# simonrw/rust-tensorflow-serving2

Measured on AMD Instinct MI355X. Metric: Predict RPCs/sec + p50 latency, ResNet-50 batch=1/32 at 1/2/4/8 MI355X, higher is better.
Workload: dtype bf16

## Files before the change

rust_tensorflow_serving2_amd/graph/fused.py:

```python
from __future__ import annotations

import os
from typing import Dict, List, Optional, Sequence, Set, Tuple

import numpy as np
import torch
import torch.nn.functional as F

from ..utils import tensors as T
from . import ops as O
from .ir import Graph, Node
from .placement import to_device, zeros

BF16 = torch.bfloat16


def _const(g: Graph, ref) -> Optional[torch.Tensor]:
    n = g.nodes.get(ref[0])
    if n is None or n.op != "Const" or n.value is None:
        return None
    v = n.value[ref[1]] if ref[1] < len(n.value) else None
    return v if isinstance(v, torch.Tensor) else None


# ... 686 lines not shown
        if not (self.use_hip and x.is_cuda and x.dim() == 4):
            return pool(ctx, node, conv(ctx, node, [x]))
        from ..ops import ACT, hip
        pt, pb, pl, pr = conv.pads_for(x.shape[1], x.shape[2])
        hc = (x.shape[1] + pt + pb - conv.kh) // conv.sh + 1
        wc = (x.shape[2] + pl + pr - conv.kw) // conv.sw + 1
        if pool.padding == "SAME":
            (ppt, ppb), (ppl, ppr) = O.tf_same_pads(hc, 3, 2), O.tf_same_pads(wc, 3, 2)
        else:
            ppt = ppb = ppl = ppr = 0
        kw = {}
        if pool.post is not None:
            sc, sh, act = pool.post
            kw = dict(post_scale=sc, post_shift=sh, post_act=ACT[act])
        x = x.contiguous() if x.dtype == torch.bfloat16 else x.float().contiguous()
        return [hip().stem_pool(x, conv.w, conv.b, pt, pb, pl, pr, ACT[conv.act],
                                ppt, ppb, ppl, ppr, **kw)]


O.OPS["_StemPool"] = _impl_op

CHAIN_SHAPES_ALL = {(64, 256, 64), (64, 256, 128), (128, 512, 128), (128, 512, 256)}
CHAIN_SHAPES_STAGE1 = {(64, 256, 64), (64, 256, 128)}
CHAIN_SHAPES_DEFAULT = CHAIN_SHAPES_ALL


class ChainConv:

    children = ("a", "b")

    def __init__(self, a: FusedConv, b: FusedConv):
        self.a, self.b = a, b
        self.use_hip = a.use_hip and b.use_hip
        self.name = a.name

    def __call__(self, ctx, node, ins):
        x = O.to_torch(ins[0])
        res = O.to_torch(ins[1]) if len(ins) > 1 else None
        a, b = self.a, self.b

        def split():
            y1 = a(ctx, node, ins)[0]
            return [y1, b(ctx, node, [y1])[0]]
        if not (self.use_hip and x.is_cuda and x.dim() == 4 and x.shape[-1] == a.cin):
            return split()
        from ..ops import ACT, hip, tuned_choice
        xb = _to_bf16(x).contiguous()
        rb = None if res is None else _to_bf16(res).contiguous()

        def chained():
            return list(hip().conv_chain(xb, a.w, a.b, rb, ACT[a.act], b.w, b.b, ACT[b.act]))
        key = ("chain", tuple(x.shape), a.cout, b.cout, res is not None, a.act, b.act)
        dflt = 1 if (a.cin, a.cout, b.cout) in CHAIN_SHAPES_STAGE1 else 0
        pick = tuned_choice(key, {1: chained, 0: split}, default=dflt)
        return chained() if pick == 1 else split()


O.OPS["_ChainConv"] = _impl_op
O.OPS["_FusedMatMulLN"] = _impl_op

_PASSTHROUGH = ("Identity", "Squeeze", "Reshape")


def fuse_classifier_head(g, order, fed, fetch_refs, device, opts):
    c = _Ctx(g, order, fed, fetch_refs, device, opts)

    def single(node) -> bool:
        return node.name not in c.fetch_nodes and len(c.cons.get(node.name, [])) == 1

    def walk(ref, chain):
        n = g.nodes.get(ref[0])
        while n is not None and n.op in _PASSTHROUGH and ref[1] == 0 and single(n) and n.inputs:
            chain.append(n)
            ref = n.inputs[0]
            n = g.nodes.get(ref[0])
        return ref, n
# ... 344 lines not shown
            g.nodes[cn].inputs[pos] = new_ref
        p.ctrl = _merge_ctrl([p, bn] + ([out_node] if out_node is not bn else []))
        del g.nodes[bn.name]
        if out_node is not bn:
            del g.nodes[out_node.name]
        c.refresh()


def _chainable_1x1(impl) -> bool:
    return (isinstance(impl, FusedConv) and impl.kh == 1 and impl.kw == 1 and impl.sh == 1 and impl.sw == 1 and
            not impl.c4 and impl.post is None and impl.act in ("relu", "none") and
            (impl.padding != "EXPLICIT" or not any(impl.pads)))


def fuse_conv_chain(g, order, fed, fetch_refs, device, opts):
    import os
    mode = os.environ.get("TFSERVE_CONV_CHAIN", "1")
    shapes = CHAIN_SHAPES_STAGE1 if os.environ.get("TFSERVE_CONV_CHAIN_SHAPES") == "stage1" else CHAIN_SHAPES_ALL
    c = _Ctx(g, order, fed, fetch_refs, device, opts)
    if mode == "0" or (not c.use_hip and mode != "force"):
        return
    for name in order:
        p = g.nodes.get(name)
        if p is None or p.op != "_FusedConv2D" or name in c.fetch_nodes:
            continue
        a = p.attrs["_impl"]
        if not _chainable_1x1(a):
            continue
        cons = c.cons.get(name, [])
        if any(i != 0 for _c, _p, i in cons):
            continue
        bs = [g.nodes[cn] for cn, pos, _i in cons
              if pos == 0 and g.nodes[cn].op == "_FusedConv2D" and len(g.nodes[cn].inputs) == 1 and
              cn not in c.fetch_nodes and _chainable_1x1(g.nodes[cn].attrs["_impl"])]
        if len(bs) != 1:
            continue
        bnode = bs[0]
        b = bnode.attrs["_impl"]
        if b.cin != a.cout or (a.cin, a.cout, b.cout) not in shapes:
            continue
        chain = ChainConv(a, b)
        p.op = "_ChainConv"
        p.attrs = {"_impl": chain}
        for cn, pos, _i in c.cons.get(bnode.name, []):
            g.nodes[cn].inputs[pos] = (name, 1)
        p.ctrl = _merge_ctrl([p, bnode])
        del g.nodes[bnode.name]
        c.refresh()


def default_passes(options=None):
    from .patterns import bert_passes, late_passes
    return [fuse_pools, fuse_softmax_argmax] + bert_passes() + [fuse_conv, fuse_dual_conv, fuse_post_activation,
                                                                 fuse_stem_pool, fuse_matmul,
                                                                 fuse_classifier_head, fuse_dense_softmax,
                                                                 fuse_conv_chain] + late_passes() + \
        [fuse_matmul_layernorm, defer_layernorm, release_weight_sources]
```

rust_tensorflow_serving2_amd/kernels/bindings.cpp:

```cpp
#include <cstdlib>
#include <algorithm>
#include <torch/extension.h>
#include <ATen/hip/impl/HIPGuardImplMasqueradingAsCUDA.h>
#include <ATen/hip/impl/HIPStreamMasqueradingAsCUDA.h>

#include "launch.h"
#include "cgemm.h"

namespace {

using torch::Tensor;

hipStream_t cur_stream(const Tensor& t) {
  return c10::hip::getCurrentHIPStreamMasqueradingAsCUDA(t.device().index()).stream();
}

void check(hipError_t e, const char* what) {
  TORCH_CHECK(e == hipSuccess, what, ": ", hipGetErrorString(e));
}

bool is_cgemm_cfg(int64_t cfg) {
  return cfg >= 0 && cfg < (1 << 20) && tfsk::cgemm_cfg_id(int(cfg));
}

// ... 407 lines not shown
  const int Hc = (H + PT + PB - 7) / 2 + 1, Wc = (W + PL + PR - 7) / 2 + 1;
  TORCH_CHECK(Hc >= 1 && Wc >= 1, "stem_pool: input smaller than the filter");
  const int Hp = (Hc + PPT + PPB - 3) / 2 + 1, Wp = (Wc + PPL + PPR - 3) / 2 + 1;
  TORCH_CHECK(Hp >= 1 && Wp >= 1, "stem_pool: conv output smaller than the pool window");
  Tensor y = torch::empty({N, Hp, Wp, cout}, x.options().dtype(at::kBFloat16));
  const float* sc = nullptr;
  const float* sh = nullptr;
  if (post_scale.has_value()) {
    TORCH_CHECK(post_shift.has_value(), "post_scale needs post_shift");
    need(*post_scale, at::kFloat, "post_scale");
    need(*post_shift, at::kFloat, "post_shift");
    TORCH_CHECK(post_scale->numel() == cout && post_shift->numel() == cout, "post scale / shift must have cout entries");
    sc = post_scale->data_ptr<float>();
    sh = post_shift->data_ptr<float>();
  }
  check(tfsk::stem_pool_launch(xin.data_ptr(), xb16, bf16p(w), int(w.size(1)), bias.data_ptr<float>(), bf16p_mut(y), N,
                               H, W, C, cout, int(PT), int(PL), Hc, Wc, int(PPT), int(PPL), Hp, Wp, int(act), sc, sh,
                               int(post_act), cur_stream(x)), "stem_pool");
  return y;
}

std::vector<Tensor> conv_chain(const Tensor& x, const Tensor& w1, const Tensor& b1,
                               const c10::optional<Tensor>& residual, int64_t act1, const Tensor& w2,
                               const Tensor& b2, int64_t act2) {
  need(x, at::kBFloat16, "x");
  need(w1, at::kBFloat16, "w1");
  need(w2, at::kBFloat16, "w2");
  need(b1, at::kFloat, "b1");
  need(b2, at::kFloat, "b2");
  TORCH_CHECK(x.dim() == 4, "conv_chain: x must be NHWC");
  const int K1 = x.size(3), N1 = w1.size(0), N2 = w2.size(0);
  TORCH_CHECK(w1.dim() == 2 && w2.dim() == 2 && w1.size(1) >= K1 && w2.size(1) >= N1 && w1.size(1) % 8 == 0 &&
                  w2.size(1) % 8 == 0, "conv_chain: w1 [N1][>= K1], w2 [N2][>= N1]");
  TORCH_CHECK(tfsk::conv_chain_supported(K1, N1, N2), "conv_chain: unsupported shape K1=", K1, " N1=", N1, " N2=", N2);
  TORCH_CHECK(b1.numel() == N1 && b2.numel() == N2, "conv_chain: bias sizes");
  TORCH_CHECK(w1.device() == x.device() && w2.device() == x.device() && b1.device() == x.device() &&
                  b2.device() == x.device(), "conv_chain: tensors on different devices");
  const uint16_t* rp = nullptr;
  if (residual.has_value()) {
    need(*residual, at::kBFloat16, "residual");
    TORCH_CHECK(residual->dim() == 4 && residual->size(0) == x.size(0) && residual->size(1) == x.size(1) &&
                    residual->size(2) == x.size(2) && residual->size(3) == N1, "conv_chain: residual [n][h][w][N1]");
    rp = bf16p(*residual);
  }
  c10::hip::HIPGuardMasqueradingAsCUDA guard(x.device());
  const int M = x.size(0) * x.size(1) * x.size(2);
  Tensor y1 = torch::empty({x.size(0), x.size(1), x.size(2), N1}, x.options());
  Tensor y2 = torch::empty({x.size(0), x.size(1), x.size(2), N2}, x.options());
  check(tfsk::conv_chain_launch(bf16p(x), bf16p(w1), int(w1.size(1)), b1.data_ptr<float>(), rp, bf16p_mut(y1),
                                bf16p(w2), int(w2.size(1)), b2.data_ptr<float>(), bf16p_mut(y2), M, K1, N1, N2,
                                int(act1), int(act2), cur_stream(x)),
        "conv_chain");
  return {y1, y2};
}

Tensor global_avgpool(const Tensor& x, const c10::optional<Tensor>& out) {
  need(x, at::kBFloat16, "x");
  TORCH_CHECK(x.dim() == 4 && x.size(3) % 8 == 0, "global_avgpool: NHWC with C % 8 == 0");
  c10::hip::HIPGuardMasqueradingAsCUDA guard(x.device());
  const int N = x.size(0), HW = x.size(1) * x.size(2), C = x.size(3);
  Tensor y = out.has_value() ? *out : torch::empty({N, C}, x.options());
  need(y, at::kBFloat16, "out");
  check(tfsk::global_avgpool_nhwc_launch(bf16p(x), bf16p_mut(y), N, HW, C, cur_stream(x)), "gap");
  return y;
}

std::vector<Tensor> softmax_argmax(const Tensor& logits, bool want_probs, bool want_classes,
                                   const c10::optional<Tensor>& probs_out,
                                   const c10::optional<Tensor>& classes_out) {
  TORCH_CHECK(logits.is_cuda() && logits.dim() >= 1 && logits.stride(-1) == 1 &&
                  (logits.is_contiguous() || logits.dim() == 2),
              "logits must be a GPU tensor with unit column stride (contiguous, or 2-D with a row stride)");
  const bool bf = logits.scalar_type() == at::kBFloat16;
  TORCH_CHECK(bf || logits.scalar_type() == at::kFloat, "logits must be f32 or bf16");
// ... 243 lines not shown
                "mask strides exceed the mask tensor");
    mb = mask_bias->data_ptr<float>();
  }
  Tensor y = out.has_value() ? *out : torch::empty({B, S, heads * D}, qkv.options());
  need(y, at::kBFloat16, "out");
  check(tfsk::attention_launch(bf16p(qkv), mb, bf16p_mut(y), B, S, heads, D, float(scale), mask_bstride,
                               mask_qstride, cur_stream(qkv)),
        "attention");
  return y;
}

}

PYBIND11_MODULE(TORCH_EXTENSION_NAME, m) {
  m.doc() = "gfx950 HIP kernels (MFMA implicit-GEMM conv/GEMM, attention, norms, pooling)";
  m.def("conv2d", &conv2d, "NHWC implicit-GEMM conv (+bias +residual +act)", py::arg("x"), py::arg("w"),
        py::arg("bias"), py::arg("residual"), py::arg("kh"), py::arg("kw"), py::arg("sh"), py::arg("sw"),
        py::arg("pt"), py::arg("pb"), py::arg("pl"), py::arg("pr"), py::arg("act") = 0, py::arg("cfg") = 0,
        py::arg("out") = py::none(), py::arg("out_f32") = false, py::arg("splits") = 1,
        py::arg("post_scale") = py::none(), py::arg("post_shift") = py::none(), py::arg("post_act") = 0,
        py::arg("out2") = py::none(), py::arg("post_only") = false);
  m.def("conv_chain", &conv_chain, "expand 1x1 (+residual, act) -> next reduce 1x1 (+act) in one kernel",
        py::arg("x"), py::arg("w1"), py::arg("b1"), py::arg("residual"), py::arg("act1"), py::arg("w2"),
        py::arg("b2"), py::arg("act2"));
  m.def("conv_chain_supported", [](int64_t k1, int64_t n1, int64_t n2) {
    return tfsk::conv_chain_supported(int(k1), int(n1), int(n2));
  });
  m.def("conv2d_dual", &conv2d_dual, "act(conv1x1(h) + conv1x1_stride(x) + bias) as one K-concatenated GEMM",
        py::arg("h"), py::arg("x"), py::arg("w"), py::arg("bias"), py::arg("sh"), py::arg("sw"), py::arg("act") = 0,
        py::arg("cfg") = 36, py::arg("out") = py::none(), py::arg("splits") = 1,
        py::arg("post_scale") = py::none(), py::arg("post_shift") = py::none(), py::arg("post_act") = 0,
        py::arg("out2") = py::none(), py::arg("post_only") = false);
  m.def("linear_lnx", &linear_lnx,
        "GEMM whose A / residual rows are LayerNorm inputs (statistics as partials), optionally "
        "returning its own rows' partials: {y, partials}",
        py::arg("x"), py::arg("w"), py::arg("bias"), py::arg("residual"), py::arg("act"), py::arg("cfg"),
        py::arg("out_f32") = false, py::arg("out") = py::none(), py::arg("a_st") = py::none(),
        py::arg("a_colsum") = py::none(), py::arg("a_eps") = 1e-12, py::arg("r_st") = py::none(),
        py::arg("r_gamma") = py::none(), py::arg("r_beta") = py::none(), py::arg("r_eps") = 1e-12,
        py::arg("stats") = false);
  m.def("linear", &linear,"x @ w^T (+bias +residual +act)", py::arg("x"), py::arg("w"), py::arg("bias"),
        py::arg("residual") = py::none(), py::arg("act") = 0, py::arg("cfg") = 0, py::arg("out_f32") = false,
        py::arg("alpha") = 1.0, py::arg("out") = py::none(), py::arg("splits") = 1);
  m.def("stem_pool", &stem_pool, py::arg("x"), py::arg("w"), py::arg("bias"), py::arg("pt"), py::arg("pb"),
        py::arg("pl"), py::arg("pr"), py::arg("act"), py::arg("ppt"), py::arg("ppb"), py::arg("ppl"), py::arg("ppr"),
        py::arg("post_scale") = py::none(), py::arg("post_shift") = py::none(), py::arg("post_act") = 0);
  m.def("maxpool", &maxpool, py::arg("x"), py::arg("kh"), py::arg("kw"), py::arg("sh"), py::arg("sw"),
        py::arg("pt"), py::arg("pb"), py::arg("pl"), py::arg("pr"), py::arg("out") = py::none(),
        py::arg("post_scale") = py::none(), py::arg("post_shift") = py::none(), py::arg("post_act") = 0);
  m.def("global_avgpool", &global_avgpool, py::arg("x"), py::arg("out") = py::none());
// ... 97 lines not shown
```

rust_tensorflow_serving2_amd/kernels/chain.hip:

```cpp
#include "gemm_common.h"

namespace tfsk {
namespace {

using namespace gemm;

struct ChainArgs {
  const uint16_t* x;
  const uint16_t* w1;
  const float* b1;
  const uint16_t* res;
  uint16_t* y1;
  const uint16_t* w2;
  const float* b2;
  uint16_t* y2;
  int M, ldw1, ldw2;
  float lo1, lo2;
};

constexpr int kBM = 64, kNT = 256, kStgLd = 68;

template <int K1, int N1, int N2>
struct CH {
  static constexpr int KT1 = K1 / KT, KT2 = N1 / KT;
  static constexpr int A_BYTES = KT1 * kBM * KT * 2;
  static constexpr int W1_BYTES = KT1 * N1 * KT * 2;
  static constexpr int P1 = A_BYTES + W1_BYTES;
  static constexpr int CHAIN = KT2 * kBM * KT * 2;
  static constexpr int STG = 4 * 16 * kStgLd * 4;
  static constexpr int S2 = N2 <= 128 ? 3 : 2;
  static constexpr int W2_SLOT = N2 * KT * 2;
  static constexpr int RING_OFF = CHAIN;
  static constexpr int P23 = CHAIN + (STG > S2 * W2_SLOT ? STG : S2 * W2_SLOT);
  static constexpr int LDS = P1 > P23 ? P1 : P23;
  static constexpr int WN1 = N1 / 4, TN1 = WN1 / 16, U1 = WN1 / 64;
  static constexpr int WN2 = N2 / 2, TN2 = WN2 / 16;
  static constexpr int UW2 = WN2 < 64 ? WN2 : 64, U2 = WN2 / UW2;
  static constexpr int APW = KT1 * (kBM / 8) / 4, W1PW = KT1 * (N1 / 8) / 4, W2PW = N2 / 32;
  static_assert(K1 % KT == 0 && N1 % 256 == 0 && N2 % 64 == 0, "chain shape");
  static_assert(LDS <= 160 * 1024, "LDS budget");
  static_assert((S2 - 2) * W2PW < 64, "vmcnt range");
};

template <int K1, int N1, int N2>
__global__ __launch_bounds__(256, 1) void conv_chain_kernel(ChainArgs p) {
  using G = CH<K1, N1, N2>;
  extern __shared__ __attribute__((aligned(16))) char smem[];
  typedef __attribute__((address_space(3))) void* lds_ptr_t;
  const int tid = threadIdx.x, lane = tid & 63;
  const int wid = __builtin_amdgcn_readfirstlane(tid >> 6);
  const int fr = lane & 15, fq = lane >> 4;
  const int prow = lane >> 3;
  const uint32_t kc = uint32_t(((lane & 7) ^ prow) * 8);
  const int m0 = xcd_remap(blockIdx.x, gridDim.x) * kBM;
  const int M = p.M;

  const __amdgpu_buffer_rsrc_t rsX = __builtin_amdgcn_make_buffer_rsrc(
      const_cast<uint16_t*>(p.x), 0, int(long(M) * K1 * 2), 0x00020000);
  const __amdgpu_buffer_rsrc_t rsW1 = __builtin_amdgcn_make_buffer_rsrc(
      const_cast<uint16_t*>(p.w1), 0, int(long(N1) * p.ldw1 * 2), 0x00020000);
  const __amdgpu_buffer_rsrc_t rsW2 = __builtin_amdgcn_make_buffer_rsrc(
      const_cast<uint16_t*>(p.w2), 0, int(long(N2) * p.ldw2 * 2), 0x00020000);

#pragma unroll
  for (int j = 0; j < G::APW; ++j) {
    const int q = wid * G::APW + j;
    const int kt = q / (kBM / 8), pc = q % (kBM / 8);
    const int m = m0 + pc * 8 + prow;
    const uint32_t v = m < M ? (uint32_t(m) * K1 + uint32_t(kt * KT) + kc) * 2u : kOOB;
    __builtin_amdgcn_raw_ptr_buffer_load_lds(rsX, (lds_ptr_t)(smem + kt * kBM * KT * 2 + pc * 1024), 16, v, 0, 0, 0);
  }
#pragma unroll
  for (int j = 0; j < G::W1PW; ++j) {
    const int q = wid * G::W1PW + j;
    const int kt = q / (N1 / 8), pc = q % (N1 / 8);
    const int n = pc * 8 + prow;
    const uint32_t v = (uint32_t(n) * uint32_t(p.ldw1) + uint32_t(kt * KT) + kc) * 2u;
    __builtin_amdgcn_raw_ptr_buffer_load_lds(rsW1, (lds_ptr_t)(smem + G::A_BYTES + kt * N1 * KT * 2 + pc * 1024), 16,
                                             v, 0, 0, 0);
  }

  const int c8 = lane & 7, rl = lane >> 3;
  float4 bias1[G::U1][2];
#pragma unroll
  for (int c = 0; c < G::U1; ++c) {
    const int n = wid * G::WN1 + c * 64 + c8 * 8;
    bias1[c][0] = *reinterpret_cast<const float4*>(p.b1 + n);
    bias1[c][1] = *reinterpret_cast<const float4*>(p.b1 + n + 4);
  }
  const __amdgpu_buffer_rsrc_t rsR = __builtin_amdgcn_make_buffer_rsrc(
      const_cast<uint16_t*>(p.res), 0, p.res ? int(long(M) * N1 * 2) : 0, 0x00020000);
  u32x4 rr[4][G::U1][2];
#pragma unroll
// ... 165 lines not shown
#pragma unroll
      for (int k = 0; k < IT2; ++k) {
        const int item = lane + 64 * k;
        const int rloc = item / CPR2, cc = item % CPR2;
        const float* src = stg + rloc * kStgLd + cc * 8;
        const float4 lo = *reinterpret_cast<const float4*>(src);
        const float4 hi = *reinterpret_cast<const float4*>(src + 4);
        const int n = wn2 * G::WN2 + c * G::UW2 + cc * 8;
        const u32x4 b0 = b2v[c][k][0], b1 = b2v[c][k][1];
        auto f = [](uint32_t u) { return __uint_as_float(u); };
        u32x4 ov;
        ov.x = pack_bf16x2(fmaxf(lo.x + f(b0.x), p.lo2), fmaxf(lo.y + f(b0.y), p.lo2));
        ov.y = pack_bf16x2(fmaxf(lo.z + f(b0.z), p.lo2), fmaxf(lo.w + f(b0.w), p.lo2));
        ov.z = pack_bf16x2(fmaxf(hi.x + f(b1.x), p.lo2), fmaxf(hi.y + f(b1.y), p.lo2));
        ov.w = pack_bf16x2(fmaxf(hi.z + f(b1.z), p.lo2), fmaxf(hi.w + f(b1.w), p.lo2));
        const int m = m0 + wm2 * 32 + i * 16 + rloc;
        __builtin_amdgcn_raw_buffer_store_b128(ov, rsY2, m < M ? (uint32_t(m) * N2 + uint32_t(n)) * 2u : kOOB, 0, 0);
      }
      __builtin_amdgcn_wave_barrier();
    }
  }
}

template <int K1, int N1, int N2>
hipError_t launch_chain(const ChainArgs& a, hipStream_t s) {
  using G = CH<K1, N1, N2>;
  hipError_t e = ensure_dyn_lds(reinterpret_cast<const void*>(&conv_chain_kernel<K1, N1, N2>), G::LDS);
  if (e != hipSuccess) return e;
  const int tiles = (a.M + kBM - 1) / kBM;
  hipLaunchKernelGGL((conv_chain_kernel<K1, N1, N2>), dim3(tiles), dim3(kNT), G::LDS, s, a);
  return hipGetLastError();
}

}

bool conv_chain_supported(int K1, int N1, int N2) {
  return (K1 == 64 && N1 == 256 && (N2 == 64 || N2 == 128)) || (K1 == 128 && N1 == 512 && (N2 == 128 || N2 == 256));
}

hipError_t conv_chain_launch(const uint16_t* x, const uint16_t* w1, int ldw1, const float* b1, const uint16_t* res,
                             uint16_t* y1, const uint16_t* w2, int ldw2, const float* b2, uint16_t* y2, int M, int K1,
                             int N1, int N2, int act1, int act2, hipStream_t s) {
  if (M <= 0) return hipSuccess;
  if (!conv_chain_supported(K1, N1, N2) || ldw1 < K1 || ldw1 % 8 || ldw2 < N1 || ldw2 % 8) return hipErrorInvalidValue;
  if ((act1 != kActNone && act1 != kActRelu) || (act2 != kActNone && act2 != kActRelu)) return hipErrorInvalidValue;
  if (long(M) * N1 * 2 >= 0x7fffffffL) return hipErrorInvalidValue;
  ChainArgs a{x, w1, b1, res, y1, w2, b2, y2, M, ldw1, ldw2, act1 == kActRelu ? 0.f : -INFINITY,
              act2 == kActRelu ? 0.f : -INFINITY};
  if (K1 == 64 && N1 == 256 && N2 == 64) return launch_chain<64, 256, 64>(a, s);
  if (K1 == 64 && N1 == 256 && N2 == 128) return launch_chain<64, 256, 128>(a, s);
  if (K1 == 128 && N1 == 512 && N2 == 128) return launch_chain<128, 512, 128>(a, s);
  return launch_chain<128, 512, 256>(a, s);
}

}
```

rust_tensorflow_serving2_amd/kernels/halo.hip:

```cpp
#include <algorithm>
#include <type_traits>

#include "gemm_common.h"
#include "cgemm.h"

namespace tfsk {

namespace {

using namespace gemm;

__device__ __forceinline__ int halo_key(int lin) { return lin & 7; }

template <int BM, int BN, int WGM, int WGN, int HR, int S_>
struct HG {
  static constexpr int NW = WGM * WGN, NT = 64 * NW;
  static constexpr int WM = BM / WGM, WN = BN / WGN;
  static constexpr int TM = WM / 16, TN = WN / 16;
  static constexpr int HPW = HR / (8 * NW);
  static constexpr int BPW = BN / (8 * NW);
  static constexpr int S = S_;
  static_assert(S == 3 || S == 9, "ring depth must divide the 9 taps (static slots)");
  static constexpr int HALO_B = HR * 128;
  static constexpr int B_B = BN * 128;
// ... 337 lines not shown
  trace_stamp(p, 2);

  halo_epilogue<BM, BN, G::NT, G::TM, G::TN, G::WM, G::WN>(p, acc, smem, h0, w0, img, n0, wm, wn, tid, bias0,
                                                              bias1);
  trace_stamp(p, 3);
}

constexpr int kPersistBM = 128, kPersistBN = 64, kPersistHR = 192;
struct HPs {
  static constexpr int BM = kPersistBM, BN = kPersistBN, HR = kPersistHR;
  static constexpr int WGM = 4, WGN = 2, NW = 8, NT = 512;
  static constexpr int WM = BM / WGM, WN = BN / WGN, TM = WM / 16, TN = WN / 16;
  static constexpr int HPW = HR / (8 * NW), BPW = BN / (8 * NW);
  static constexpr int B_B = BN * 128, HALO_B = HR * 128;
  static constexpr int CB_LD = BN + 8;
  static constexpr int STG_B = BM * CB_LD * 2;
  static constexpr int OFF_HALO = 9 * B_B, OFF_STG = OFF_HALO + 2 * HALO_B;
  static constexpr int LDS = OFF_STG + STG_B;
  static constexpr int kStores = BM * (BN / 8) / NT;
  static_assert(HPW * 8 * NW == HR && BPW == 1 && kStores * NT == BM * (BN / 8), "persistent halo split");
  static_assert(LDS <= 160 * 1024, "LDS budget");
};

__global__ __launch_bounds__(512, 1) void halo_persist_kernel(IGemmArgs p, int ntiles) {
  using G = HPs;
  constexpr int BM = G::BM, BN = G::BN;
  extern __shared__ __attribute__((aligned(16))) char smem_raw[];
  char* const smem = reinterpret_cast<char*>(smem_raw);
  typedef __attribute__((address_space(3))) void* lds_ptr_t;

  const int TH = p.TH, TW = p.TW, HW2 = TW + 2;
  const int Ho = p.Ho, Wo = p.Wo, H = p.H, W = p.W, C = p.C;
  const int tph = (Ho + TH - 1) / TH, tpw = (Wo + TW - 1) / TW;
  const int TI = p.TI > 1 ? p.TI : 1, nimg = p.M / (Ho * Wo);
  const int HB = (TH + 2) * HW2, hrows = TI * HB;
  const int tid = threadIdx.x, lane = tid & 63;
  const int wid = __builtin_amdgcn_readfirstlane(tid >> 6);
  const int wm = wid / G::WGN, wn = wid % G::WGN;
  const int prow = lane >> 3;
  const int fr = lane & 15, fq = lane >> 4;

  const __amdgpu_buffer_rsrc_t rsA =
      __builtin_amdgcn_make_buffer_rsrc(const_cast<void*>(p.a), 0, int(p.a_bytes), 0x00020000);
  const __amdgpu_buffer_rsrc_t rsB =
      __builtin_amdgcn_make_buffer_rsrc(const_cast<uint16_t*>(p.b), 0, int(p.b_bytes), 0x00020000);
  const __amdgpu_buffer_rsrc_t rsO =
      __builtin_amdgcn_make_buffer_rsrc(p.out, 0, int(long(p.M) * p.ldc * 2), 0x00020000);
  const bool use_b = p.bias != nullptr;
  const __amdgpu_buffer_rsrc_t rsb =
      __builtin_amdgcn_make_buffer_rsrc(const_cast<float*>(p.bias), 0, use_b ? BN * 4 : 0, 0x00020000);

  float bj[G::TN];
#pragma unroll
  for (int j = 0; j < G::TN; ++j)
    bj[j] = __uint_as_float(__builtin_amdgcn_raw_buffer_load_b32(rsb, uint32_t(wn * G::WN + j * 16 + fr) * 4u, 0, 0));
  const float alpha = p.alpha;
  gemm::wait_vmcnt<0>();

  {
    const uint32_t kc = uint32_t(((lane & 7) ^ prow) * 8);
    const int n = wid * 8 + prow;
    const uint32_t boff = (uint32_t(n) * uint32_t(p.ldb) + kc) * 2u;
#pragma unroll
// ... 25 lines not shown
  };

  int hrow0[G::TM], kpx0[G::TM];
#pragma unroll
  for (int i = 0; i < G::TM; ++i) {
    const int px = wm * G::WM + i * 16 + fr;
    const int ii = px / (TH * TW), p2 = px - ii * (TH * TW);
    const int ph = p2 / TW;
    hrow0[i] = px < TI * TH * TW ? ii * HB + ph * HW2 + (p2 - ph * TW) : 0;
    kpx0[i] = px;
  }
  const uint32_t rb0 = uint32_t(((wn * G::WN + fr) * KT + ((fq ^ (fr & 7)) * 8)) * 2);
  const uint32_t rb1 = uint32_t(((wn * G::WN + fr) * KT + (((4 + fq) ^ (fr & 7)) * 8)) * 2);
  constexpr int CPRB = BN / 8;
  uint16_t* const Cb = reinterpret_cast<uint16_t*>(smem + G::OFF_STG);

  int t = blockIdx.x;
  if (t < ntiles) issue_halo(t, 0);
  for (int k = 0; t < ntiles; t += gridDim.x, ++k) {
    const int b = k & 1;
    if (k == 0) gemm::wait_vmcnt<0>();
    else gemm::wait_vmcnt<G::kStores>();
    gemm::lds_barrier();
    const int tn = t + gridDim.x;
    if (tn < ntiles) issue_halo(tn, b ^ 1);
    __builtin_amdgcn_sched_barrier(0);

    f32x4 acc[G::TM][G::TN];
#pragma unroll
    for (int i = 0; i < G::TM; ++i)
#pragma unroll
      for (int j = 0; j < G::TN; ++j) acc[i][j] = f32x4{0.f, 0.f, 0.f, 0.f};
    const char* hb = smem + G::OFF_HALO + b * G::HALO_B;
    struct TapFrags {
      bf16x8 a[2][G::TM], b[2][G::TN];
    };
    auto load_tap = [&](TapFrags& f, int u) __attribute__((always_inline)) {
      const int tap_off = (u / 3) * HW2 + (u % 3), tap_key = (u / 3) * TW + (u % 3);
      const char* sb = smem + u * G::B_B;
#pragma unroll
      for (int kk = 0; kk < 2; ++kk) {
#pragma unroll
        for (int i = 0; i < G::TM; ++i) {
          const int hr = hrow0[i] + tap_off;
          const uint32_t addr = uint32_t(hr) * 128u + ((uint32_t((kk * 4 + fq) ^ halo_key(kpx0[i] + tap_key))) << 4);
          f.a[kk][i] = *reinterpret_cast<const bf16x8*>(hb + addr);
        }
#pragma unroll
        for (int j = 0; j < G::TN; ++j)
          f.b[kk][j] = *reinterpret_cast<const bf16x8*>(sb + (kk ? rb1 : rb0) + j * 16 * KT * 2);
      }
    };
    TapFrags fr2[2];
    load_tap(fr2[0], 0);
#pragma unroll
    for (int u = 0; u < 9; ++u) {
      __builtin_amdgcn_sched_barrier(0);
      if (u < 8) load_tap(fr2[(u + 1) & 1], u + 1);
      __builtin_amdgcn_sched_barrier(0);
      const TapFrags& f = fr2[u & 1];
#pragma unroll
      for (int kk = 0; kk < 2; ++kk)
#pragma unroll
        for (int i = 0; i < G::TM; ++i)
#pragma unroll
          for (int j = 0; j < G::TN; ++j)
            acc[i][j] = __builtin_amdgcn_mfma_f32_16x16x32_bf16(f.a[kk][i], f.b[kk][j], acc[i][j], 0, 0, 0);
    }
    __builtin_amdgcn_sched_barrier(0);

    auto stage = [&](auto act_tag) __attribute__((always_inline)) {
      constexpr int ACT = decltype(act_tag)::value;
#pragma unroll
      for (int i = 0; i < G::TM; ++i)
#pragma unroll
        for (int j = 0; j < G::TN; ++j)
#pragma unroll
          for (int r = 0; r < 4; ++r) {
            const float v = act_fn<ACT>(acc[i][j][r] * alpha + bj[j] + 0.f);
            Cb[(wm * G::WM + i * 16 + fq * 4 + r) * G::CB_LD + wn * G::WN + j * 16 + fr] =
                __builtin_bit_cast(uint16_t, static_cast<__bf16>(v));
          }
    };
    switch (p.act) {
      case kActRelu: stage(std::integral_constant<int, kActRelu>{}); break;
      case kActGeluTanh: stage(std::integral_constant<int, kActGeluTanh>{}); break;
      case kActTanh: stage(std::integral_constant<int, kActTanh>{}); break;
      default: stage(std::integral_constant<int, kActNone>{}); break;
    }
    gemm::lds_barrier();
    {
      int r_ = t;
      const int tw = r_ % tpw;
      r_ /= tpw;
      const int th = r_ % tph;
      const int img = (r_ / tph) * TI;
      const int h0 = th * TH, w0 = tw * TW;
#pragma unroll
      for (int it = 0; it < G::kStores; ++it) {
        const int c = tid + it * G::NT, row = c / CPRB, ch = c - row * CPRB;
        int m = -1;
        if (row < TI * TH * TW) {
          const int ii = row / (TH * TW), r2 = row - ii * (TH * TW);
          const int ph = r2 / TW, pw = r2 - ph * TW;
          const int h = h0 + ph, w = w0 + pw;
          if (h < Ho && w < Wo && img + ii < nimg) m = ((img + ii) * Ho + h) * Wo + w;
        }
        const uint32_t off = m >= 0 ? (uint32_t(m) * uint32_t(p.ldc) + uint32_t(ch * 8)) * 2u : kOOB;
        const u32x4 v = *reinterpret_cast<const u32x4*>(Cb + row * G::CB_LD + ch * 8);
        __builtin_amdgcn_raw_buffer_store_b128(v, rsO, off, 0, 0);
      }
    }
  }
  gemm::wait_vmcnt<0>();
}



bool pick_block(int Ho, int Wo, int BM, int HR, int& TH, int& TW) {
  long best_tiles = -1, best_halo = 0;
  for (int tw = 1; tw <= Wo; ++tw) {
    int th = BM / tw < Ho ? BM / tw : Ho;
    while (th >= 1 && (th + 2) * (tw + 2) > HR) --th;
    if (th < 1) continue;
    const int nh = (Ho + th - 1) / th, nw = (Wo + tw - 1) / tw;
    const int bh = (Ho + nh - 1) / nh, bw = (Wo + nw - 1) / nw;
    const long tiles = long(nh) * nw;
    const long halo = long(bh + 2) * (bw + 2);
    if (best_tiles < 0 || tiles < best_tiles || (tiles == best_tiles && halo < best_halo)) {
      best_tiles = tiles;
      best_halo = halo;
      TH = bh;
      TW = bw;
    }
  }
  return best_tiles > 0;
}
// ... 32 lines not shown

hipError_t launch_halo_persist(const IGemmArgs& a0, hipStream_t s) {
  using G = HPs;
  IGemmArgs a = a0;
  if (a.C != KT || a.N != G::BN || a.splits > 1 || a.residual != nullptr || a.out2 != nullptr || a.out_f32 ||
      a.out == nullptr || a.act == kActGeluErf || epi_f32_env() || a.counters != nullptr || a.ldc % 8)
    return hipErrorInvalidValue;
  if (long(a.M) * a.ldc * 2 >= 0x7fffffffL) return hipErrorInvalidValue;
  if (!pick_block(a.Ho, a.Wo, G::BM, G::HR, a.TH, a.TW)) return hipErrorInvalidValue;
  a.TI = pick_images(a, G::BM, G::HR);
  const int nimg = a.M / (a.Ho * a.Wo);
  const long tiles = long((nimg + a.TI - 1) / a.TI) * ((a.Ho + a.TH - 1) / a.TH) * ((a.Wo + a.TW - 1) / a.TW);
  if (tiles == 0) return hipSuccess;
  if (tiles >= (1L << 30)) return hipErrorInvalidValue;
  static int cus = 0;
  if (cus == 0) {
    int dev = 0, n = 0;
    if (hipGetDevice(&dev) != hipSuccess || hipDeviceGetAttribute(&n, hipDeviceAttributeMultiprocessorCount, dev) !=
                                                hipSuccess || n <= 0)
      n = 256;
    cus = n;
  }
  const int grid = int(tiles < cus ? tiles : cus);
  hipError_t e = ensure_dyn_lds(reinterpret_cast<const void*>(&halo_persist_kernel), G::LDS);
  if (e != hipSuccess) return e;
  hipLaunchKernelGGL(halo_persist_kernel, dim3(unsigned(grid)), dim3(G::NT), G::LDS, s, a, int(tiles));
  return hipGetLastError();
}

constexpr int kHBM[kNumHaloConfigs] = {256, 128, 128, 64, 256, 64, 64, 128, 256, 128, 128};
constexpr int kHBN[kNumHaloConfigs] = {64, 128, 64, 64, 128, 128, 64, 64, 64, 64, 64};
constexpr int kHHR[kNumHaloConfigs] = {320, 192, 192, 128, 320, 128, 128, 192, 320, 192, 192};

int halo_cfg_index(int cfg) {
  if (cfg >= kHaloCfgBase && cfg < kHaloCfgBase + kNumHaloConfigs) return cfg - kHaloCfgBase;
  if (cfg >= kHaloPfCfgBase && cfg < kHaloPfCfgBase + kNumHaloConfigs) return cfg - kHaloPfCfgBase;
  return -1;
}

}

long halo_tiles(const IGemmArgs& a0, int cfg) {
  IGemmArgs a = a0;
  a.epi_f32 = epi_f32_env();
  if (cfg == kHaloPersistCfg) return 0;
  const int c = halo_cfg_index(cfg);
  if (c < 0) return 0;
  if (!pick_block(a.Ho, a.Wo, kHBM[c], kHHR[c], a.TH, a.TW)) return 0;
  const int nimg = a.M / (a.Ho * a.Wo);
// ... 51 lines not shown
```

rust_tensorflow_serving2_amd/kernels/launch.h:

```cpp
#pragma once
#include <hip/hip_runtime.h>
#include <stdint.h>

namespace tfsk {

struct IGemmArgs {
  const void* a;
  const uint16_t* b;
  int M, N, K;
  int lda, ldb;
  int H, W, C, KH, KW, SH, SW, PT, PL, Ho, Wo;
  const float* bias;
  const uint16_t* residual;
  int ldr;
  int act;
  void* out;
  int ldc;
  int out_f32;
  float alpha;
  int splits;
  int kt_per_split;
  float* ws;
  int64_t a_bytes;
  int64_t b_bytes;
// ... 30 lines not shown
int64_t splitk_counters_pending();
int64_t splitk_counters_captured_in_use();

enum AMode : int { kADense = 0, kAIm2col = 1, kAStemF32 = 2, kAStem7x7x3 = 3, kAC4 = 4, kADual = 5 };

hipError_t ingest_c4_launch(const float* x, uint16_t* y, int64_t pixels, int C, hipStream_t stream);

hipError_t ingest_c4_pad_launch(const float* x, uint16_t* y, int N, int H, int W, int C, int Hp, int Wp, int pt,
                               int pl, hipStream_t stream);

hipError_t splitk_reduce_launch(const IGemmArgs& args, hipStream_t stream);

constexpr int kNumIGemmConfigs = 17;
int igemm_config_bm(int cfg);
int igemm_config_bn(int cfg);
int igemm_config_stages(int cfg);
int igemm_config_bk(int cfg);
hipError_t igemm_launch(const IGemmArgs& args, int a_mode, int cfg, hipStream_t stream);

hipError_t stem_pool_launch(const void* x, bool x_bf16, const uint16_t* w, int ldw, const float* bias, uint16_t* y,
                            int N, int H, int W, int C, int cout, int pt, int pl, int Hc, int Wc, int ppt, int ppl,
                            int Hp, int Wp, int act, const float* pscale, const float* pshift, int pact,
                            hipStream_t s);
bool conv_chain_supported(int K1, int N1, int N2);
hipError_t conv_chain_launch(const uint16_t* x, const uint16_t* w1, int ldw1, const float* b1, const uint16_t* res,
                             uint16_t* y1, const uint16_t* w2, int ldw2, const float* b2, uint16_t* y2, int M, int K1,
                             int N1, int N2, int act1, int act2, hipStream_t s);
hipError_t maxpool_nhwc_launch(const uint16_t* x, uint16_t* y, int N, int H, int W, int C,
                               int KH, int KW, int SH, int SW, int PT, int PL, int Ho, int Wo,
                               hipStream_t stream, const float* scale = nullptr, const float* shift = nullptr,
                               int act = 0);
hipError_t global_avgpool_nhwc_launch(const uint16_t* x, uint16_t* y, int N, int HW, int C,
                                      hipStream_t stream);
hipError_t classifier_head_launch(const uint16_t* x, const uint16_t* w, const float* bias, float* ws,
                                  float* probs, int64_t* classes, int M, int HW, int K, int Np, int N,
                                  hipStream_t s, int* counter = nullptr, float* probs_h = nullptr,
                                  int64_t* classes_h = nullptr);
size_t classifier_head_ws_floats(int M, int K, int Np);
bool classifier_head_one_launch(int M, int HW, int K, int Np, int N);
hipError_t dense_softmax_launch(const float* x, int ldx, const uint16_t* w, int ldw, const float* bias,
                                float* probs, int rows, int N, int K, hipStream_t s);
hipError_t key_mask_adder_launch(const void* m, int is_int, float one, float scale, float* out, int64_t n,
                                 hipStream_t s);
hipError_t softmax_argmax_launch(const void* logits, int in_bf16, float* probs, int64_t* classes,
                                 int rows, int cols, long ld, hipStream_t stream);
hipError_t cast_f32_bf16_launch(const float* x, uint16_t* y, int64_t n, hipStream_t stream);
hipError_t cast_bf16_f32_launch(const uint16_t* x, float* y, int64_t n, hipStream_t stream);
int epi_f32_env();
hipError_t h2d_rows_launch(const void* host, void* dev, int64_t bytes, hipStream_t stream);

// ... 28 lines not shown
```

Before: 55980.

## Chain dual-source 1x1 projection conv into following reduce conv

Extends the chained 1x1 conv kernel so the first GEMM can take two input sources, K-concatenated (the dual conv that merges the bottleneck expand with the shortcut projection). The first stage-1 block's projection output then feeds the next block's reduce conv in one kernel, saving a launch and a round trip of the 256-channel intermediate through memory. It is enabled by default for the (128,256,64) shape through the tuned choice. The halo persistent kernel also gains a compile-time trace variant so the untraced path carries no trace branches.

```diff
diff --git a/rust_tensorflow_serving2_amd/graph/fused.py b/rust_tensorflow_serving2_amd/graph/fused.py
--- a/rust_tensorflow_serving2_amd/graph/fused.py
+++ b/rust_tensorflow_serving2_amd/graph/fused.py
@@ -732,6 +732,7 @@
 
 CHAIN_SHAPES_ALL = {(64, 256, 64), (64, 256, 128), (128, 512, 128), (128, 512, 256)}
 CHAIN_SHAPES_STAGE1 = {(64, 256, 64), (64, 256, 128)}
+CHAIN_SHAPES_DUAL = {(128, 256, 64)}
 CHAIN_SHAPES_DEFAULT = CHAIN_SHAPES_ALL
 
 
@@ -739,19 +740,25 @@
 
     children = ("a", "b")
 
-    def __init__(self, a: FusedConv, b: FusedConv):
+    def __init__(self, a, b: FusedConv):
         self.a, self.b = a, b
+        self.dual = isinstance(a, FusedDualConv)
         self.use_hip = a.use_hip and b.use_hip
         self.name = a.name
+        if self.dual:
+            from types import SimpleNamespace
+            self.subs = [(a, SimpleNamespace(op="_FusedDualConv")), (b, SimpleNamespace(op="_FusedConv2D"))]
 
     def __call__(self, ctx, node, ins):
         x = O.to_torch(ins[0])
-        res = O.to_torch(ins[1]) if len(ins) > 1 else None
         a, b = self.a, self.b
 
         def split():
             y1 = a(ctx, node, ins)[0]
             return [y1, b(ctx, node, [y1])[0]]
+        if self.dual:
+            return self._call_dual(x, O.to_torch(ins[1]), split)
+        res = O.to_torch(ins[1]) if len(ins) > 1 else None
         if not (self.use_hip and x.is_cuda and x.dim() == 4 and x.shape[-1] == a.cin):
             return split()
         from ..ops import ACT, hip, tuned_choice
@@ -762,6 +769,21 @@
             return list(hip().conv_chain(xb, a.w, a.b, rb, ACT[a.act], b.w, b.b, ACT[b.act]))
         key = ("chain", tuple(x.shape), a.cout, b.cout, res is not None, a.act, b.act)
         dflt = 1 if (a.cin, a.cout, b.cout) in CHAIN_SHAPES_STAGE1 else 0
+        pick = tuned_choice(key, {1: chained, 0: split}, default=dflt)
+        return chained() if pick == 1 else split()
+
+    def _call_dual(self, h, x, split):
+        a, b = self.a, self.b
+        if not (self.use_hip and h.is_cuda and h.dim() == 4 and x.dim() == 4 and h.shape[:3] == x.shape[:3] and
+                h.shape[-1] == a.c1 and x.shape[-1] == a.c2):
+            return split()
+        from ..ops import ACT, hip, tuned_choice
+        hb, xb = _to_bf16(h).contiguous(), _to_bf16(x).contiguous()
+
+        def chained():
+            return list(hip().conv_chain(hb, a.w, a.b, None, ACT[a.act], b.w, b.b, ACT[b.act], x2=xb))
+        key = ("chain", tuple(h.shape), a.cout, b.cout, ("dual", a.c2), a.act, b.act)
+        dflt = 1 if (a.c1 + a.c2, a.cout, b.cout) in CHAIN_SHAPES_DUAL else 0
         pick = tuned_choice(key, {1: chained, 0: split}, default=dflt)
         return chained() if pick == 1 else split()
 
@@ -1152,10 +1174,14 @@
         return
     for name in order:
         p = g.nodes.get(name)
-        if p is None or p.op != "_FusedConv2D" or name in c.fetch_nodes:
+        if p is None or p.op not in ("_FusedConv2D", "_FusedDualConv") or name in c.fetch_nodes:
             continue
         a = p.attrs["_impl"]
-        if not _chainable_1x1(a):
+        dual = p.op == "_FusedDualConv"
+        if dual:
+            if not (a.use_hip and a.sh == a.sw == 1 and a.post is None and a.act in ("relu", "none")):
+                continue
+        elif not _chainable_1x1(a):
             continue
         cons = c.cons.get(name, [])
         if any(i != 0 for _c, _p, i in cons):
@@ -1167,7 +1193,8 @@
             continue
         bnode = bs[0]
         b = bnode.attrs["_impl"]
-        if b.cin != a.cout or (a.cin, a.cout, b.cout) not in shapes:
+        shape = (a.c1 + a.c2 if dual else a.cin, a.cout, b.cout)
+        if b.cin != a.cout or shape not in (CHAIN_SHAPES_DUAL if dual else shapes):
             continue
         chain = ChainConv(a, b)
         p.op = "_ChainConv"
diff --git a/rust_tensorflow_serving2_amd/kernels/bindings.cpp b/rust_tensorflow_serving2_amd/kernels/bindings.cpp
--- a/rust_tensorflow_serving2_amd/kernels/bindings.cpp
+++ b/rust_tensorflow_serving2_amd/kernels/bindings.cpp
@@ -453,17 +453,30 @@
 
 std::vector<Tensor> conv_chain(const Tensor& x, const Tensor& w1, const Tensor& b1,
                                const c10::optional<Tensor>& residual, int64_t act1, const Tensor& w2,
-                               const Tensor& b2, int64_t act2) {
+                               const Tensor& b2, int64_t act2, const c10::optional<Tensor>& x2) {
   need(x, at::kBFloat16, "x");
   need(w1, at::kBFloat16, "w1");
   need(w2, at::kBFloat16, "w2");
   need(b1, at::kFloat, "b1");
   need(b2, at::kFloat, "b2");
   TORCH_CHECK(x.dim() == 4, "conv_chain: x must be NHWC");
-  const int K1 = x.size(3), N1 = w1.size(0), N2 = w2.size(0);
+  const bool dual = x2.has_value();
+  const int Ka = x.size(3);
+  const uint16_t* x2p = nullptr;
+  if (dual) {
+    need(*x2, at::kBFloat16, "x2");
+    TORCH_CHECK(x2->dim() == 4 && x2->size(0) == x.size(0) && x2->size(1) == x.size(1) && x2->size(2) == x.size(2),
+                "conv_chain: x2 must have x's n, h, w");
+    TORCH_CHECK(Ka % 64 == 0 && x2->size(3) % 64 == 0 && x2->size(3) > 0,
+                "conv_chain: both sources' channels must be multiples of 64");
+    TORCH_CHECK(x2->device() == x.device(), "conv_chain: tensors on different devices");
+    x2p = bf16p(*x2);
+  }
+  const int K1 = Ka + (dual ? int(x2->size(3)) : 0), N1 = w1.size(0), N2 = w2.size(0);
   TORCH_CHECK(w1.dim() == 2 && w2.dim() == 2 && w1.size(1) >= K1 && w2.size(1) >= N1 && w1.size(1) % 8 == 0 &&
                   w2.size(1) % 8 == 0, "conv_chain: w1 [N1][>= K1], w2 [N2][>= N1]");
-  TORCH_CHECK(tfsk::conv_chain_supported(K1, N1, N2), "conv_chain: unsupported shape K1=", K1, " N1=", N1, " N2=", N2);
+  TORCH_CHECK(tfsk::conv_chain_supported(K1, N1, N2, dual), "conv_chain: unsupported shape K1=", K1, " N1=", N1,
+              " N2=", N2, dual ? " (dual)" : "");
   TORCH_CHECK(b1.numel() == N1 && b2.numel() == N2, "conv_chain: bias sizes");
   TORCH_CHECK(w1.device() == x.device() && w2.device() == x.device() && b1.device() == x.device() &&
                   b2.device() == x.device(), "conv_chain: tensors on different devices");
@@ -480,7 +493,7 @@
   Tensor y2 = torch::empty({x.size(0), x.size(1), x.size(2), N2}, x.options());
   check(tfsk::conv_chain_launch(bf16p(x), bf16p(w1), int(w1.size(1)), b1.data_ptr<float>(), rp, bf16p_mut(y1),
                                 bf16p(w2), int(w2.size(1)), b2.data_ptr<float>(), bf16p_mut(y2), M, K1, N1, N2,
-                                int(act1), int(act2), cur_stream(x)),
+                                int(act1), int(act2), cur_stream(x), x2p, Ka),
         "conv_chain");
   return {y1, y2};
 }
@@ -770,10 +783,10 @@
         py::arg("out2") = py::none(), py::arg("post_only") = false);
   m.def("conv_chain", &conv_chain, "expand 1x1 (+residual, act) -> next reduce 1x1 (+act) in one kernel",
         py::arg("x"), py::arg("w1"), py::arg("b1"), py::arg("residual"), py::arg("act1"), py::arg("w2"),
-        py::arg("b2"), py::arg("act2"));
-  m.def("conv_chain_supported", [](int64_t k1, int64_t n1, int64_t n2) {
-    return tfsk::conv_chain_supported(int(k1), int(n1), int(n2));
-  });
+        py::arg("b2"), py::arg("act2"), py::arg("x2") = py::none());
+  m.def("conv_chain_supported", [](int64_t k1, int64_t n1, int64_t n2, bool dual) {
+    return tfsk::conv_chain_supported(int(k1), int(n1), int(n2), dual);
+  }, py::arg("k1"), py::arg("n1"), py::arg("n2"), py::arg("dual") = false);
   m.def("conv2d_dual", &conv2d_dual, "act(conv1x1(h) + conv1x1_stride(x) + bias) as one K-concatenated GEMM",
         py::arg("h"), py::arg("x"), py::arg("w"), py::arg("bias"), py::arg("sh"), py::arg("sw"), py::arg("act") = 0,
         py::arg("cfg") = 36, py::arg("out") = py::none(), py::arg("splits") = 1,
diff --git a/rust_tensorflow_serving2_amd/kernels/chain.hip b/rust_tensorflow_serving2_amd/kernels/chain.hip
--- a/rust_tensorflow_serving2_amd/kernels/chain.hip
+++ b/rust_tensorflow_serving2_amd/kernels/chain.hip
@@ -7,6 +7,7 @@
 
 struct ChainArgs {
   const uint16_t* x;
+  const uint16_t* x2;
   const uint16_t* w1;
   const float* b1;
   const uint16_t* res;
@@ -15,6 +16,7 @@
   const float* b2;
   uint16_t* y2;
   int M, ldw1, ldw2;
+  int K1a;
   float lo1, lo2;
 };
 
@@ -42,7 +44,7 @@
   static_assert((S2 - 2) * W2PW < 64, "vmcnt range");
 };
 
-template <int K1, int N1, int N2>
+template <int K1, int N1, int N2, bool DUAL = false>
 __global__ __launch_bounds__(256, 1) void conv_chain_kernel(ChainArgs p) {
   using G = CH<K1, N1, N2>;
   extern __shared__ __attribute__((aligned(16))) char smem[];
@@ -55,8 +57,11 @@
   const int m0 = xcd_remap(blockIdx.x, gridDim.x) * kBM;
   const int M = p.M;
 
+  const int Ka = DUAL ? p.K1a : K1;
   const __amdgpu_buffer_rsrc_t rsX = __builtin_amdgcn_make_buffer_rsrc(
-      const_cast<uint16_t*>(p.x), 0, int(long(M) * K1 * 2), 0x00020000);
+      const_cast<uint16_t*>(p.x), 0, int(long(M) * Ka * 2), 0x00020000);
+  const __amdgpu_buffer_rsrc_t rsX2 = __builtin_amdgcn_make_buffer_rsrc(
+      const_cast<uint16_t*>(DUAL ? p.x2 : p.x), 0, DUAL ? int(long(M) * (K1 - Ka) * 2) : 0, 0x00020000);
   const __amdgpu_buffer_rsrc_t rsW1 = __builtin_amdgcn_make_buffer_rsrc(
       const_cast<uint16_t*>(p.w1), 0, int(long(N1) * p.ldw1 * 2), 0x00020000);
   const __amdgpu_buffer_rsrc_t rsW2 = __builtin_amdgcn_make_buffer_rsrc(
@@ -67,8 +72,14 @@
     const int q = wid * G::APW + j;
     const int kt = q / (kBM / 8), pc = q % (kBM / 8);
     const int m = m0 + pc * 8 + prow;
-    const uint32_t v = m < M ? (uint32_t(m) * K1 + uint32_t(kt * KT) + kc) * 2u : kOOB;
-    __builtin_amdgcn_raw_ptr_buffer_load_lds(rsX, (lds_ptr_t)(smem + kt * kBM * KT * 2 + pc * 1024), 16, v, 0, 0, 0);
+    if (DUAL && kt * KT >= Ka) {
+      const uint32_t v = m < M ? (uint32_t(m) * uint32_t(K1 - Ka) + uint32_t(kt * KT - Ka) + kc) * 2u : kOOB;
+      __builtin_amdgcn_raw_ptr_buffer_load_lds(rsX2, (lds_ptr_t)(smem + kt * kBM * KT * 2 + pc * 1024), 16, v, 0, 0,
+                                               0);
+    } else {
+      const uint32_t v = m < M ? (uint32_t(m) * uint32_t(Ka) + uint32_t(kt * KT) + kc) * 2u : kOOB;
+      __builtin_amdgcn_raw_ptr_buffer_load_lds(rsX, (lds_ptr_t)(smem + kt * kBM * KT * 2 + pc * 1024), 16, v, 0, 0, 0);
+    }
   }
 #pragma unroll
   for (int j = 0; j < G::W1PW; ++j) {
@@ -280,31 +291,36 @@
   }
 }
 
-template <int K1, int N1, int N2>
+template <int K1, int N1, int N2, bool DUAL = false>
 hipError_t launch_chain(const ChainArgs& a, hipStream_t s) {
   using G = CH<K1, N1, N2>;
-  hipError_t e = ensure_dyn_lds(reinterpret_cast<const void*>(&conv_chain_kernel<K1, N1, N2>), G::LDS);
+  hipError_t e = ensure_dyn_lds(reinterpret_cast<const void*>(&conv_chain_kernel<K1, N1, N2, DUAL>), G::LDS);
   if (e != hipSuccess) return e;
   const int tiles = (a.M + kBM - 1) / kBM;
-  hipLaunchKernelGGL((conv_chain_kernel<K1, N1, N2>), dim3(tiles), dim3(kNT), G::LDS, s, a);
+  hipLaunchKernelGGL((conv_chain_kernel<K1, N1, N2, DUAL>), dim3(tiles), dim3(kNT), G::LDS, s, a);
   return hipGetLastError();
 }
 
 }
 
-bool conv_chain_supported(int K1, int N1, int N2) {
+bool conv_chain_supported(int K1, int N1, int N2, bool dual) {
+  static_assert(CH<128, 256, 64>::LDS <= 80 * 1024, "two workgroups per CU");
+  if (dual) return K1 == 128 && N1 == 256 && N2 == 64;
   return (K1 == 64 && N1 == 256 && (N2 == 64 || N2 == 128)) || (K1 == 128 && N1 == 512 && (N2 == 128 || N2 == 256));
 }
 
 hipError_t conv_chain_launch(const uint16_t* x, const uint16_t* w1, int ldw1, const float* b1, const uint16_t* res,
                              uint16_t* y1, const uint16_t* w2, int ldw2, const float* b2, uint16_t* y2, int M, int K1,
-                             int N1, int N2, int act1, int act2, hipStream_t s) {
+                             int N1, int N2, int act1, int act2, hipStream_t s, const uint16_t* x2, int K1a) {
   if (M <= 0) return hipSuccess;
-  if (!conv_chain_supported(K1, N1, N2) || ldw1 < K1 || ldw1 % 8 || ldw2 < N1 || ldw2 % 8) return hipErrorInvalidValue;
+  const bool dual = x2 != nullptr;
+  if (dual && (K1a <= 0 || K1a >= K1 || K1a % KT || (K1 - K1a) % KT)) return hipErrorInvalidValue;
+  if (!conv_chain_supported(K1, N1, N2, dual) || ldw1 < K1 || ldw1 % 8 || ldw2 < N1 || ldw2 % 8) return hipErrorInvalidValue;
   if ((act1 != kActNone && act1 != kActRelu) || (act2 != kActNone && act2 != kActRelu)) return hipErrorInvalidValue;
   if (long(M) * N1 * 2 >= 0x7fffffffL) return hipErrorInvalidValue;
-  ChainArgs a{x, w1, b1, res, y1, w2, b2, y2, M, ldw1, ldw2, act1 == kActRelu ? 0.f : -INFINITY,
+  ChainArgs a{x, x2, w1, b1, res, y1, w2, b2, y2, M, ldw1, ldw2, dual ? K1a : K1, act1 == kActRelu ? 0.f : -INFINITY,
               act2 == kActRelu ? 0.f : -INFINITY};
+  if (dual) return launch_chain<128, 256, 64, true>(a, s);
   if (K1 == 64 && N1 == 256 && N2 == 64) return launch_chain<64, 256, 64>(a, s);
   if (K1 == 64 && N1 == 256 && N2 == 128) return launch_chain<64, 256, 128>(a, s);
   if (K1 == 128 && N1 == 512 && N2 == 128) return launch_chain<128, 512, 128>(a, s);
diff --git a/rust_tensorflow_serving2_amd/kernels/halo.hip b/rust_tensorflow_serving2_amd/kernels/halo.hip
--- a/rust_tensorflow_serving2_amd/kernels/halo.hip
+++ b/rust_tensorflow_serving2_amd/kernels/halo.hip
@@ -383,6 +383,7 @@
   static_assert(LDS <= 160 * 1024, "LDS budget");
 };
 
+template <bool TRACE>
 __global__ __launch_bounds__(512, 1) void halo_persist_kernel(IGemmArgs p, int ntiles) {
   using G = HPs;
   constexpr int BM = G::BM, BN = G::BN;
@@ -400,6 +401,7 @@
   const int wm = wid / G::WGN, wn = wid % G::WGN;
   const int prow = lane >> 3;
   const int fr = lane & 15, fq = lane >> 4;
+  if constexpr (TRACE) trace_stamp(p, 0);
 
   const __amdgpu_buffer_rsrc_t rsA =
       __builtin_amdgcn_make_buffer_rsrc(const_cast<void*>(p.a), 0, int(p.a_bytes), 0x00020000);
@@ -471,6 +473,8 @@
     if (k == 0) gemm::wait_vmcnt<0>();
     else gemm::wait_vmcnt<G::kStores>();
     gemm::lds_barrier();
+    if constexpr (TRACE)
+      if (k < 2) trace_stamp(p, k == 0 ? 1 : 4);
     const int tn = t + gridDim.x;
     if (tn < ntiles) issue_halo(tn, b ^ 1);
     __builtin_amdgcn_sched_barrier(0);
@@ -517,6 +521,8 @@
             acc[i][j] = __builtin_amdgcn_mfma_f32_16x16x32_bf16(f.a[kk][i], f.b[kk][j], acc[i][j], 0, 0, 0);
     }
     __builtin_amdgcn_sched_barrier(0);
+    if constexpr (TRACE)
+      if (k < 2) trace_stamp(p, k == 0 ? 2 : 5);
 
     auto stage = [&](auto act_tag) __attribute__((always_inline)) {
       constexpr int ACT = decltype(act_tag)::value;
@@ -560,8 +566,11 @@
         __builtin_amdgcn_raw_buffer_store_b128(v, rsO, off, 0, 0);
       }
     }
+    if constexpr (TRACE)
+      if (k == 0) trace_stamp(p, 3);
   }
   gemm::wait_vmcnt<0>();
+  if constexpr (TRACE) trace_stamp(p, 6);
 }
 
 
@@ -640,9 +649,15 @@
     cus = n;
   }
   const int grid = int(tiles < cus ? tiles : cus);
-  hipError_t e = ensure_dyn_lds(reinterpret_cast<const void*>(&halo_persist_kernel), G::LDS);
+  if (a.trace != nullptr) {
+    hipError_t e = ensure_dyn_lds(reinterpret_cast<const void*>(&halo_persist_kernel<true>), G::LDS);
+    if (e != hipSuccess) return e;
+    hipLaunchKernelGGL(halo_persist_kernel<true>, dim3(unsigned(grid)), dim3(G::NT), G::LDS, s, a, int(tiles));
+    return hipGetLastError();
+  }
+  hipError_t e = ensure_dyn_lds(reinterpret_cast<const void*>(&halo_persist_kernel<false>), G::LDS);
   if (e != hipSuccess) return e;
-  hipLaunchKernelGGL(halo_persist_kernel, dim3(unsigned(grid)), dim3(G::NT), G::LDS, s, a, int(tiles));
+  hipLaunchKernelGGL(halo_persist_kernel<false>, dim3(unsigned(grid)), dim3(G::NT), G::LDS, s, a, int(tiles));
   return hipGetLastError();
 }
 
diff --git a/rust_tensorflow_serving2_amd/kernels/launch.h b/rust_tensorflow_serving2_amd/kernels/launch.h
--- a/rust_tensorflow_serving2_amd/kernels/launch.h
+++ b/rust_tensorflow_serving2_amd/kernels/launch.h
@@ -76,10 +76,11 @@
                             int N, int H, int W, int C, int cout, int pt, int pl, int Hc, int Wc, int ppt, int ppl,
                             int Hp, int Wp, int act, const float* pscale, const float* pshift, int pact,
                             hipStream_t s);
-bool conv_chain_supported(int K1, int N1, int N2);
+bool conv_chain_supported(int K1, int N1, int N2, bool dual = false);
 hipError_t conv_chain_launch(const uint16_t* x, const uint16_t* w1, int ldw1, const float* b1, const uint16_t* res,
                              uint16_t* y1, const uint16_t* w2, int ldw2, const float* b2, uint16_t* y2, int M, int K1,
-                             int N1, int N2, int act1, int act2, hipStream_t s);
+                             int N1, int N2, int act1, int act2, hipStream_t s, const uint16_t* x2 = nullptr,
+                             int K1a = 0);
 hipError_t maxpool_nhwc_launch(const uint16_t* x, uint16_t* y, int N, int H, int W, int C,
                                int KH, int KW, int SH, int SW, int PT, int PL, int Ho, int Wo,
                                hipStream_t stream, const float* scale = nullptr, const float* shift = nullptr,
```

New measurement: 56850 (median of 6 runs). 1.02x the previous value.
